# maybeLx/MVSFormerPlusPlus

Hardware: NVIDIA H100
Metric: depth-maps/sec (hot path: FMT + 4-stage cascade) (higher is better)
Workload: dtype f32

## Files before the change

mvsformerplusplus_b200/csrc/conv3d_tc.cu:

```cuda
#include "conv3d_tc.cuh"

#include <type_traits>

#include "linear_tc.cuh"
#include "wgmma.cuh"

namespace mvsf {

using namespace gmma;

namespace c3 {
constexpr int THREADS = 384, MAX_STAGES = 8;
template <int MODE, int NT>
struct Geo {
  static constexpr int TW = 8 * NT, TH = 16;
  static constexpr int PR = MODE == CONV_S1 ? TH + 2 : TH + 1;
  static constexpr int PC = MODE == CONV_S1 ? TW + 2 : TW + 1;
  static constexpr int NSUB = MODE == CONV_S2 ? 4 : 1;
  static constexpr uint32_t SUB_BYTES = PR * PC * 16;
  static constexpr uint32_t PAIR = (2 * SUB_BYTES + 127) / 128 * 128;
  static constexpr uint32_t OCT_BYTES = NSUB * PAIR;
  static constexpr uint32_t PITCH = PC * 16;
};
__host__ __device__ inline int npad(int cout) { return cout < 16 ? 16 : cout; }
__host__ __device__ inline uint32_t slab_bytes(int mode, int cout) { return (uint32_t)npad(cout) * (mode == DECONV_S2 ? 1024u : 576u); }

struct alignas(64) Maps { CUtensorMap m[4]; };
}

struct DepthTaps { int n, kd[3], id[3]; };
template <int MODE>
__device__ __forceinline__ DepthTaps depth_taps(int od, int SD, int ID) {
  DepthTaps t;
  t.n = 0;
#pragma unroll
  for (int kd = 0; kd < 3; ++kd) {
    int id;
    bool ok = true;
    if (MODE == CONV_S1) id = od + kd - 1;
    else if (MODE == CONV_S2) id = od * SD + kd - 1;
    else {
      const int num = od + 1 - kd;
      if (SD == 1) id = num;
      else { ok = (num & 1) == 0; id = num >> 1; }
    }
    if (ok && id >= 0 && id < ID) { t.kd[t.n] = kd; t.id[t.n] = id; ++t.n; }
  }
  return t;
}

template <int OUT, int NPAD>
__device__ __forceinline__ float conv_epilogue_frag(const ConvTcArgs& a, const float* acc, int h, int q, bool valid, size_t vox) {
  const int COUT = a.COUT;
  float prob = 0.f;
#pragma unroll
  for (int b = 0; b < NPAD / 8; ++b) {
    const int c = 8 * b + 2 * q;
    if (8 * b >= COUT) continue;
    const float2 b2 = *reinterpret_cast<const float2*>(a.bias + c);
    float x0 = fmaxf(acc[4 * b + 2 * h] + b2.x, 0.f), x1 = fmaxf(acc[4 * b + 2 * h + 1] + b2.y, 0.f);
    if (!valid) continue;
    if (OUT == OUT_SPLIT) {
      if (a.skip_hi) {
        const float2 fh = __half22float2(*reinterpret_cast<const __half2*>(a.skip_hi + vox * COUT + c));
        const float2 fl = __half22float2(*reinterpret_cast<const __half2*>(a.skip_lo + vox * COUT + c));
        x0 += fh.x + fl.x;
        x1 += fh.y + fl.y;
      }
      split_store2(a.out_hi + vox * COUT + c, a.out_lo + vox * COUT + c, x0, x1);
    } else {
      const float2 s2 = *reinterpret_cast<const float2*>(a.skip32 + vox * COUT + c);
      x0 += s2.x; x1 += s2.y;
      if (OUT == OUT_F32) *reinterpret_cast<float2*>(a.out32 + vox * COUT + c) = make_float2(x0, x1);
      else prob = fmaf(x1, __ldg(a.probw + c + 1), x0 * __ldg(a.probw + c));
    }
  }
  return prob;
}

template <int NREG>
__device__ __forceinline__ void fence_acc(float (&acc)[NREG]) { fence_regs<NREG>(acc); }

template <int MODE, int NT, int OUT, int NPAD>
__global__ void __launch_bounds__(c3::THREADS, 1)
conv3d_tc_kernel(const __grid_constant__ c3::Maps maps, ConvTcArgs a, int NS, int OD, int OH, int OW, int tiles_w,
                 int tiles_h, int ntiles) {
  using G = c3::Geo<MODE, NT>;
  constexpr int PC = G::PC, NSUB = G::NSUB;
  constexpr int NCLS = MODE == DECONV_S2 ? 4 : 1;
  constexpr int ACC = NCLS * NPAD / 2;
  extern __shared__ __align__(1024) unsigned char smem[];
  const int tid = threadIdx.x, warp = tid >> 5, lane = tid & 31;
  const int CIN = a.CIN, SD = a.SD, ID = a.ID, IH = a.IH, IW = a.IW;
  const int KG = a.KG;
  const uint32_t b_bytes = c3::slab_bytes(MODE, NPAD);
  const uint32_t a_bytes = (uint32_t)KG * G::OCT_BYTES;
  const uint32_t stage_bytes = (a_bytes + b_bytes + 127u) / 128u * 128u;
  const uint32_t sbase = smem_u32(smem);
  const uint32_t bars = sbase + NS * stage_bytes;
  const uint32_t bar_full = bars, bar_empty = bars + 64;
  const int ngroups = (CIN >> 3) / KG;

  if (tid == 0) {
    for (int i = 0; i < c3::MAX_STAGES; ++i) { mbar_init(bar_full + 8 * i, 1); mbar_init(bar_empty + 8 * i, 2); }
    fence_barrier_init();
  }
  __syncthreads();

  if (warp < 4) {
    asm volatile("setmaxnreg.dec.sync.aligned.u32 40;");
    if (tid == 0) {
      uint32_t g = 0;
      for (int tile = blockIdx.x; tile < ntiles; tile += gridDim.x) {
        const int tw = tile % tiles_w, th = (tile / tiles_w) % tiles_h, od = tile / (tiles_w * tiles_h);
        const int c0h = th * 16, c0w = tw * G::TW;
        const DepthTaps dt = depth_taps<MODE>(od, SD, ID);
        for (int ds = 0; ds < dt.n; ++ds) {
          for (int grp = 0; grp < ngroups; ++grp, ++g) {
            const int s = g % NS;
            mbar_wait(bar_empty + 8 * s, (uint32_t)(((g / NS) & 1) ^ 1));
            const uint32_t st = sbase + s * stage_bytes, full = bar_full + 8 * s;
            expect_tx(full, (uint32_t)(KG * NSUB) * 2u * G::SUB_BYTES + b_bytes);
            for (int og = 0; og < KG; ++og) {
              const int c = (grp * KG + og) * 8;
#pragma unroll
              for (int sub = 0; sub < NSUB; ++sub) {
// ... 50 lines not shown
        }
      };
      wg_fence();
      if constexpr (MODE == DECONV_S2) {
        issue(0u, 0, u == 0);
        issue(16u, 4, false);
        issue((uint32_t)PC * 16u, 8, false);
        issue((uint32_t)(PC + 1) * 16u, 12, false);
      } else {
#pragma unroll
        for (int kh = 0; kh < 3; ++kh) {
#pragma unroll
          for (int kw = 0; kw < 3; ++kw) {
            int sub = 0, rs = kh, cs = kw;
            if (MODE == CONV_S2) {
              sub = (kh == 1 ? 0 : 2) + (kw == 1 ? 0 : 1);
              rs = kh == 2 ? 1 : 0; cs = kw == 2 ? 1 : 0;
            }
            issue((uint32_t)sub * G::PAIR + (uint32_t)(rs * PC + cs) * 16u, kh * 3 + kw, u == 0 && kh == 0 && kw == 0);
          }
        }
      }
      wg_commit();
      if (pend >= 0) {
        wg_wait<1>();
        release((uint32_t)pend);
      }
      pend = (int)g;
    }
    wg_wait<0>();
#pragma unroll
    for (int t = 0; t < NT; ++t) fence_acc(acc[t]);
    release((uint32_t)pend);
#pragma unroll
    for (int t = 0; t < NT; ++t)
#pragma unroll
      for (int cls = 0; cls < NCLS; ++cls)
#pragma unroll
        for (int h = 0; h < 2; ++h) {
          const int ch = th * 16 + 8 * half + 2 * wq + h;
          const int cw = tw * G::TW + t * 8 + (lane >> 2);
          int oh, ow;
          bool valid;
          if (MODE == DECONV_S2) { oh = 2 * ch + (cls >> 1); ow = 2 * cw + (cls & 1); valid = ch < IH && cw < IW; }
          else { oh = ch; ow = cw; valid = ch < OH && cw < OW; }
          const size_t vox = valid ? ((size_t)od * OH + oh) * OW + ow : 0;
          float prob = conv_epilogue_frag<OUT, NPAD>(a, acc[t] + (cls ^ (cls >> 1)) * (NPAD / 2), h, q, valid, vox);
          if (OUT == OUT_PROB) {
            prob += __shfl_xor_sync(0xffffffffu, prob, 1);
            prob += __shfl_xor_sync(0xffffffffu, prob, 2);
            if (q == 0 && valid) a.out32[vox] = prob + __ldg(a.probw + a.COUT);
          }
        }
  }
}


template <int MODE, int NT, int NPAD>
__global__ void __launch_bounds__(c3::THREADS, 1)
conv3d_col_kernel(const __grid_constant__ c3::Maps maps, ConvTcArgs a, int NS, int wres, int OH, int OW, int tiles_w,
                  int tiles_h, int DC, int nitems) {
  using G = c3::Geo<MODE, NT>;
  constexpr int PC = G::PC, NSUB = G::NSUB;
  extern __shared__ __align__(1024) unsigned char smem[];
  const int tid = threadIdx.x, warp = tid >> 5, lane = tid & 31;
  const int CIN = a.CIN, D = a.ID;
  const int KG = a.KG;
  const int ngroups = (CIN >> 3) / KG;
  const uint32_t slab = (uint32_t)NPAD * 1728u;
  const uint32_t a_bytes = (uint32_t)KG * G::OCT_BYTES;
  const uint32_t stage_bytes = (a_bytes + (wres ? 0u : slab) + 127u) / 128u * 128u;
  const uint32_t sbase = smem_u32(smem);
  const uint32_t wbase = sbase;
  const uint32_t ring = sbase + (wres ? ((uint32_t)ngroups * slab + 127u) / 128u * 128u : 0u);
  const uint32_t bars = ring + NS * stage_bytes;
  const uint32_t bar_full = bars, bar_empty = bars + 64, bar_w = bars + 128;

  if (tid == 0) {
    for (int i = 0; i < c3::MAX_STAGES; ++i) { mbar_init(bar_full + 8 * i, 1); mbar_init(bar_empty + 8 * i, 2); }
    mbar_init(bar_w, 1);
    fence_barrier_init();
  }
  __syncthreads();
  const int tiles_hw = tiles_w * tiles_h;

  if (warp < 4) {
    asm volatile("setmaxnreg.dec.sync.aligned.u32 40;");
    if (tid == 0) {
      if (wres) {
        expect_tx(bar_w, (uint32_t)ngroups * slab);
        for (int grp = 0; grp < ngroups; ++grp) bulk_load(wbase + grp * slab, a.wtc + (size_t)grp * (slab / 2), slab, bar_w);
      }
      uint32_t g = 0;
      for (int item = blockIdx.x; item < nitems; item += gridDim.x) {
        const int tw = item % tiles_w, th = (item / tiles_w) % tiles_h, ck = item / tiles_hw;
        const int c0h = th * 16, c0w = tw * G::TW;
        const int d0 = ck * DC, d1 = min(D, d0 + DC);
        const int first_id = max(d0 - 1, 0), last_id = min(d1, D - 1);
        for (int id = first_id; id <= last_id; ++id) {
          for (int grp = 0; grp < ngroups; ++grp, ++g) {
            const int s = g % NS;
            mbar_wait(bar_empty + 8 * s, (uint32_t)(((g / NS) & 1) ^ 1));
            const uint32_t st = ring + s * stage_bytes, full = bar_full + 8 * s;
            expect_tx(full, (uint32_t)(KG * NSUB) * 2u * G::SUB_BYTES + (wres ? 0u : slab));
            for (int og = 0; og < KG; ++og) {
              const int c = (grp * KG + og) * 8;
#pragma unroll
              for (int sub = 0; sub < NSUB; ++sub) {
                int w0, h0;
                if (MODE == CONV_S1) { w0 = c0w - 1; h0 = c0h - 1; }
                else { w0 = c0w - (sub & 1); h0 = c0h - (sub >> 1); }
                tma_load_5d(st + (uint32_t)(og * NSUB + sub) * G::PAIR, &maps.m[sub], c, w0, h0, id, 0, full);
              }
            }
            if (!wres) bulk_load(st + a_bytes, a.wtc + (size_t)grp * (slab / 2), slab, full);
          }
        }
      }
    }
    return;
  }
  asm volatile("setmaxnreg.inc.sync.aligned.u32 232;");
  const int half = (warp >> 2) - 1, wq = warp & 3, q = lane & 3, t128 = tid & 127;
  if (wres) mbar_wait(bar_w, 0u);
  constexpr uint32_t btile = (uint32_t)NPAD * 96u;
  constexpr uint32_t blbo = (uint32_t)NPAD * 48u;
  constexpr int SL = NPAD / 2;
  float acc[NT][3 * SL];
  auto release = [&](uint32_t gb) { if (t128 == 0) mbar_arrive(bar_empty + 8 * (gb % NS)); };
  auto epilogue = [&](int od, int th, int tw, auto third_c) {
#pragma unroll
    for (int t = 0; t < NT; ++t)
#pragma unroll
      for (int h = 0; h < 2; ++h) {
        const int ch = th * 16 + 8 * half + 2 * wq + h;
        const int cw = tw * G::TW + t * 8 + (lane >> 2);
        const bool valid = ch < OH && cw < OW;
        const size_t vox = valid ? ((size_t)od * OH + ch) * OW + cw : 0;
        conv_epilogue_frag<OUT_SPLIT, NPAD>(a, acc[t] + decltype(third_c)::value * SL, h, q, valid, vox);
      }
  };
  uint32_t g = 0;
  for (int item = blockIdx.x; item < nitems; item += gridDim.x) {
    const int tw = item % tiles_w, th = (item / tiles_w) % tiles_h, ck = item / tiles_hw;
    const int d0 = ck * DC, d1 = min(D, d0 + DC);
    const int first_id = max(d0 - 1, 0), last_id = min(d1, D - 1);
#pragma unroll
    for (int t = 0; t < NT; ++t)
#pragma unroll
      for (int i = 0; i < 3 * SL; ++i) acc[t][i] = 0.f;
    for (int id = first_id; id <= last_id; ++id) {
      int pend = -1;
      for (int grp = 0; grp < ngroups; ++grp, ++g) {
        const int s = g % NS;
        mbar_wait(bar_full + 8 * s, (uint32_t)((g / NS) & 1));
        const uint32_t sA = ring + s * stage_bytes + (uint32_t)half * 8u * G::PITCH;
        const uint32_t sB = wres ? wbase + grp * slab : ring + s * stage_bytes + a_bytes;
        wg_fence();
#pragma unroll
        for (int kh = 0; kh < 3; ++kh) {
#pragma unroll
          for (int kw = 0; kw < 3; ++kw) {
            int sub = 0, rs = kh, cs = kw;
            if (MODE == CONV_S2) {
              sub = (kh == 1 ? 0 : 2) + (kw == 1 ? 0 : 1);
              rs = kh == 2 ? 1 : 0; cs = kw == 2 ? 1 : 0;
            }
            const uint32_t aoff = sA + (uint32_t)sub * G::PAIR + (uint32_t)(rs * PC + cs) * 16u;
            const uint32_t t0 = sB + (uint32_t)(kh * 3 + kw) * 2u * btile, t1 = t0 + btile;
            const uint32_t va[3] = {KG == 1 ? aoff : aoff + G::SUB_BYTES, KG == 1 ? aoff : aoff, aoff};
            const uint32_t vl = KG == 1 ? G::SUB_BYTES : G::OCT_BYTES;
            const uint32_t vt[3] = {t0, t1, t0};
            const int nv = KG == 1 ? 2 : 3;
#pragma unroll
            for (int v = 0; v < 3; ++v) {
              if (v >= nv) break;
              const uint64_t bd = make_desc(vt[v], blbo, 128);
#pragma unroll
              for (int t = 0; t < NT; ++t) mma_ss<3 * NPAD>(acc[t], make_desc(va[v] + t * 128, vl, G::PITCH), bd, 1u);
            }
          }
        }
        wg_commit();
        if (pend >= 0) {
          wg_wait<1>();
          release((uint32_t)pend);
        }
        pend = (int)g;
      }
      wg_wait<0>();
#pragma unroll
      for (int t = 0; t < NT; ++t) fence_acc(acc[t]);
      release((uint32_t)pend);
      if (id - 1 >= d0) epilogue(id - 1, th, tw, std::integral_constant<int, 0>{});
      if (id == last_id && id <= d1 - 1) epilogue(id, th, tw, std::integral_constant<int, 1>{});
#pragma unroll
      for (int t = 0; t < NT; ++t)
#pragma unroll
        for (int i = 0; i < SL; ++i) {
          acc[t][i] = acc[t][SL + i];
          acc[t][SL + i] = acc[t][2 * SL + i];
          acc[t][2 * SL + i] = 0.f;
        }
    }
  }
}

int conv3d_tc_kg(int mode, int cin) { return (mode != CONV_S2 && cin >= 16) ? 2 : 1; }
int conv3d_tc_col(int mode, int sd, int cout) { return (mode == CONV_S1 || (mode == CONV_S2 && sd == 1)) && c3::npad(cout) <= 32; }

size_t conv3d_tc_packed_halves(int mode, int cin, int cout) {
  return (size_t)3 * (cin / 8 / conv3d_tc_kg(mode, cin)) * (c3::slab_bytes(mode, cout) / 2);
}

__global__ void conv3d_tc_pack_kernel(const float* __restrict__ w32, __half* __restrict__ out, int cin, int cout, int NPAD,
                                      int KG, int deconv, int col, size_t total) {
  size_t i = (size_t)blockIdx.x * blockDim.x + threadIdx.x;
  if (i >= total) return;
  const int e = (int)(i & 7);
  const size_t q = i >> 3;
  const int per_slab = col ? NPAD * 108 : (deconv ? NPAD * 64 : NPAD * 36);
  const int slab = (int)(q / per_slab), c = (int)(q % per_slab);
  const int ngroups = cin / 8 / KG;
  int kd = slab / ngroups, g = slab % ngroups;
  int mm, kc, n, kh = 0, kw = 0;
  bool tap = true;
  if (col) {
    g = slab;
    n = c % NPAD;
    int r = c / NPAD;
    kd = 2 - r % 3; r /= 3;
    kc = r & 1; r >>= 1;
    mm = r & 1; r >>= 1;
    kh = r / 3; kw = r % 3;
  } else if (!deconv) {
    n = c % NPAD;
    int r = c / NPAD;
    kc = r & 1; r >>= 1;
    mm = r & 1; r >>= 1;
    kh = r / 3; kw = r % 3;
  } else {
    const int tkh[4][4] = {{1, 1, 2, 2}, {-1, 1, 2, -1}, {-1, -1, 0, 0}, {-1, -1, 0, -1}};
    const int tkw[4][4] = {{1, 2, 2, 1}, {-1, 0, 0, -1}, {-1, -1, 2, 1}, {-1, -1, 0, -1}};
    const int t = c / (16 * NPAD), cc = c % (16 * NPAD);
    mm = cc / (8 * NPAD);
    kc = (cc / (4 * NPAD)) & 1;
    const int nn = cc % (4 * NPAD);
    const int b = nn / NPAD;
    n = nn % NPAD;
    kh = tkh[t][b]; kw = tkw[t][b];
    tap = kh >= 0;
  }
  const int ci = (KG == 1 ? g : g * 2 + kc) * 8 + e;
  float w = 0.f;
  if (tap && n < cout) w = w32[((size_t)((kd * 3 + kh) * 3 + kw) * cin + ci) * cout + n];
  __half hi, lo;
  split_f16(w, hi, lo);
  __half v;
  if (KG == 1) v = mm == 0 ? hi : (kc == 0 ? lo : __float2half_rn(0.f));
  else v = mm == 0 ? hi : lo;
  out[i] = v;
}

int conv3d_tc_pack(const float* w32, __half* out, int mode, int sd, int cin, int cout, cudaStream_t s) {
  MVSF_REQUIRE(w32 && out && cin % 8 == 0 && cout % 8 == 0, "conv3d_tc_pack: bad arguments");
  const size_t total = conv3d_tc_packed_halves(mode, cin, cout);
  conv3d_tc_pack_kernel<<<cdiv((long long)total, 256), 256, 0, s>>>(w32, out, cin, cout, c3::npad(cout),
                                                                     conv3d_tc_kg(mode, cin), mode == DECONV_S2 ? 1 : 0,
                                                                     conv3d_tc_col(mode, sd, cout), total);
  MVSF_LAUNCH_CHECK("conv3d_tc_pack");
  return MVSF_OK;
}

__global__ void merge_vec8_kernel(const __half* __restrict__ hi, const __half* __restrict__ lo, float* __restrict__ x, size_t n8) {
  size_t i = (size_t)blockIdx.x * blockDim.x + threadIdx.x;
  if (i >= n8) return;
// ... 82 lines not shown
  else { OD = a.ID * a.SD; OH = a.IH * 2; OW = a.IW * 2; cells_h = a.IH; cells_w = a.IW; }
  const int num_sms = device_sm_count(current_device());
  const int NPAD = c3::npad(a.COUT);
  const uint32_t b_bytes = c3::slab_bytes(MODE, a.COUT);
  const int ncls = MODE == DECONV_S2 ? 4 : 1;
  int best_nt = 0;
  double best_eff = -1.0;
  const int nts[3] = {4, 2, 1};
  size_t stage_of[5] = {0, 0, 0, 0, 0};
  for (int k = 0; k < 3; ++k) {
    const int nt = nts[k];
    const uint32_t oct = nt == 4 ? c3::Geo<MODE, 4>::OCT_BYTES : (nt == 2 ? c3::Geo<MODE, 2>::OCT_BYTES : c3::Geo<MODE, 1>::OCT_BYTES);
    const size_t stage = align_up((size_t)a.KG * oct + b_bytes, 128);
    stage_of[nt] = stage;
    if (nt * ncls * NPAD > 256 || 2 * stage + 256 > 227 * 1024) continue;
    const long long ntiles = (long long)cdiv(cells_w, 8 * nt) * cdiv(cells_h, 16) * OD;
    const double eff = (double)ntiles / (double)(cdiv(ntiles, num_sms) * (long long)num_sms);
    if (eff >= 0.85) { best_nt = nt; break; }
    if (eff > best_eff) { best_eff = eff; best_nt = nt; }
  }
  MVSF_REQUIRE(best_nt > 0, "conv3d_tc: no tile shape fits (COUT %d)", a.COUT);
  const size_t stage = stage_of[best_nt];
  int NS = (int)((227 * 1024 - 256) / stage);
  if (NS > c3::MAX_STAGES) NS = c3::MAX_STAGES;
  const size_t smem = NS * stage + 256;
  if constexpr (OUT == OUT_SPLIT) {
    if (NPAD == 32) return launch_nt<MODE, OUT, 32>(a, best_nt, NS, smem, OD, OH, OW, cells_h, cells_w, num_sms, s);
    if (NPAD == 64) return launch_nt<MODE, OUT, 64>(a, best_nt, NS, smem, OD, OH, OW, cells_h, cells_w, num_sms, s);
  }
  return launch_nt<MODE, OUT, 16>(a, best_nt, NS, smem, OD, OH, OW, cells_h, cells_w, num_sms, s);
}


template <int MODE, int NT, int NPAD>
static int launch_col_one(const ConvTcArgs& a, int NS, int wres, size_t smem, int OH, int OW, int DC, int num_sms, cudaStream_t s) {
  using G = c3::Geo<MODE, NT>;
  auto kern = conv3d_col_kernel<MODE, NT, NPAD>;
  static DeviceOnce once;
  const int dev = current_device();
  if (once.need(dev)) {
    MVSF_CUDA_OK(cudaFuncSetAttribute(kern, cudaFuncAttributeMaxDynamicSharedMemorySize, 227 * 1024));
    once.done(dev);
  }
  c3::Maps maps;
  int rc;
  if (MODE == CONV_S2) {
    for (int sub = 0; sub < 4; ++sub)
      if ((rc = make_map(&maps.m[sub], a.in_hi, a.in_lo, a.CIN, a.ID, a.IH, a.IW, 2, 2, sub >> 1, sub & 1, G::PC, G::PR))) return rc;
  } else {
    if ((rc = make_map(&maps.m[0], a.in_hi, a.in_lo, a.CIN, a.ID, a.IH, a.IW, 1, 1, 0, 0, G::PC, G::PR))) return rc;
    maps.m[1] = maps.m[2] = maps.m[3] = maps.m[0];
  }
  const int tiles_w = cdiv(OW, 8 * NT), tiles_h = cdiv(OH, 16);
  const long long nitems = (long long)tiles_w * tiles_h * cdiv(a.ID, DC);
  MVSF_REQUIRE(nitems < (1ll << 30), "conv3d_tc: volume too large");
  const int grid = (int)(nitems < num_sms ? nitems : num_sms);
  kern<<<grid, c3::THREADS, smem, s>>>(maps, a, NS, wres, OH, OW, tiles_w, tiles_h, DC, (int)nitems);
  MVSF_LAUNCH_CHECK("conv3d_col");
  return MVSF_OK;
}

template <int MODE>
static int launch_col(const ConvTcArgs& a, cudaStream_t s) {
  const int D = a.ID;
  const int OH = MODE == CONV_S1 ? a.IH : (a.IH - 1) / 2 + 1, OW = MODE == CONV_S1 ? a.IW : (a.IW - 1) / 2 + 1;
  const int num_sms = device_sm_count(current_device());
  const int NPAD = c3::npad(a.COUT);
  const int ngroups = a.CIN / 8 / a.KG;
  const size_t slab = (size_t)NPAD * 1728;
  const size_t wres_bytes = align_up(ngroups * slab, 128);
  const int wres = wres_bytes <= 112 * 1024 ? 1 : 0;
  int best_nt = 0, best_dc = 0, best_ns = 0;
  size_t best_smem = 0;
  double best_cost = 1e30;
  const int nts[3] = {4, 2, 1};
  for (int k = 0; k < 3; ++k) {
    const int nt = nts[k];
    if (3 * nt * NPAD > 128) continue;
    const uint32_t oct = nt == 4 ? c3::Geo<MODE, 4>::OCT_BYTES : (nt == 2 ? c3::Geo<MODE, 2>::OCT_BYTES : c3::Geo<MODE, 1>::OCT_BYTES);
    const size_t stage = align_up((size_t)a.KG * oct + (wres ? 0 : slab), 128);
    const size_t fixed = (wres ? wres_bytes : 0) + 256;
    int ns = (int)((227 * 1024 - fixed) / stage);
    if (ns > c3::MAX_STAGES) ns = c3::MAX_STAGES;
    if (ns < 2) continue;
    for (int div = 1; div <= 8; div *= 2) {
      const int dc = cdiv(D, div);
      if (div > 1 && dc == cdiv(D, div / 2)) continue;
      const long long items = (long long)cdiv(OW, 8 * nt) * cdiv(OH, 16) * cdiv(D, dc);
      const double eff = (double)items / (double)(cdiv(items, num_sms) * (long long)num_sms);
      const double halo_w = MODE == CONV_S1 ? (8.0 * nt + 2) / (8.0 * nt) : (16.0 * nt + 1) / (16.0 * nt);
      const double halo_d = dc >= D ? 1.0 : (dc + 2.0) / dc;
      const double cost = halo_w * halo_d / eff;
      if (cost < best_cost) { best_cost = cost; best_nt = nt; best_dc = dc; best_ns = ns; best_smem = fixed + ns * stage; }
    }
  }
  MVSF_REQUIRE(best_nt > 0, "conv3d_col: no tile shape fits (CIN %d COUT %d)", a.CIN, a.COUT);
  if (NPAD == 16) {
    if (best_nt == 2) return launch_col_one<MODE, 2, 16>(a, best_ns, wres, best_smem, OH, OW, best_dc, num_sms, s);
    return launch_col_one<MODE, 1, 16>(a, best_ns, wres, best_smem, OH, OW, best_dc, num_sms, s);
  }
  return launch_col_one<MODE, 1, 32>(a, best_ns, wres, best_smem, OH, OW, best_dc, num_sms, s);
}

int launch_conv3d_tc(const ConvTcArgs& a, int mode, int out_mode, cudaStream_t s) {
  MVSF_REQUIRE(a.in_hi && a.in_lo && a.wtc && a.bias, "conv3d_tc: null pointer");
  MVSF_REQUIRE(a.CIN % 8 == 0 && a.CIN >= 8 && a.CIN <= 64 && (a.COUT == 8 || a.COUT == 16 || a.COUT == 32 || a.COUT == 64),
               "conv3d_tc: input channels must be a multiple of 8 up to 64, output channels 8, 16, 32 or 64");
  MVSF_REQUIRE(a.SD == 1 || a.SD == 2, "conv3d_tc: depth stride must be 1 or 2");
  MVSF_REQUIRE(a.KG == conv3d_tc_kg(mode, a.CIN), "conv3d_tc: KG must be conv3d_tc_kg(mode, CIN) (it fixes the weight slab layout)");
  MVSF_REQUIRE(((uintptr_t)a.in_hi & 15) == 0 && ((uintptr_t)a.in_lo & 15) == 0 && ((uintptr_t)a.wtc & 15) == 0,
               "conv3d_tc: operands must be 16-byte aligned");
  MVSF_REQUIRE(a.col == conv3d_tc_col(mode, a.SD, a.COUT), "conv3d_tc: col must be conv3d_tc_col(mode, SD, COUT) (weight slab layout)");
  if (out_mode == OUT_SPLIT) {
    MVSF_REQUIRE(a.out_hi && a.out_lo, "conv3d_tc: split output missing");
    if (a.col) return mode == CONV_S1 ? launch_col<CONV_S1>(a, s) : launch_col<CONV_S2>(a, s);
    if (mode == CONV_S1) return launch_mode<CONV_S1, OUT_SPLIT>(a, s);
    if (mode == CONV_S2) return launch_mode<CONV_S2, OUT_SPLIT>(a, s);
    if (mode == DECONV_S2) return launch_mode<DECONV_S2, OUT_SPLIT>(a, s);
  } else if (mode == DECONV_S2 && (out_mode == OUT_F32 || out_mode == OUT_PROB)) {
    MVSF_REQUIRE(a.out32 && a.skip32 && a.COUT == 8 && (out_mode == OUT_F32 || a.probw), "conv3d_tc: fp32 output needs out32, skip32, COUT == 8");
    if (out_mode == OUT_F32) return launch_mode<DECONV_S2, OUT_F32>(a, s);
    return launch_mode<DECONV_S2, OUT_PROB>(a, s);
  }
  return fail(MVSF_ERR_INVALID, "conv3d_tc: unsupported mode %d / output %d", mode, out_mode);
}

}

using namespace mvsf;

extern "C" int mvsf_conv3d_tc_layer(int mode, int sd, const float* in, const float* w32, const float* skip, float* out,
                                    void* workspace, size_t workspace_bytes, int cin, int cout, int ID, int IH, int IW,
                                    mvsf_stream_t stream) {
  MVSF_REQUIRE(in && w32 && out && workspace && (mode >= 0 && mode <= 2) && (sd == 1 || sd == 2), "conv3d_tc_layer: bad arguments");
  MVSF_REQUIRE(cin % 8 == 0 && cout % 8 == 0, "conv3d_tc_layer: channels must be multiples of 8");
  int OD, OH, OW;
  if (mode == CONV_S1) { OD = ID; OH = IH; OW = IW; }
  else if (mode == CONV_S2) { OD = (ID - 1) / sd + 1; OH = (IH - 1) / 2 + 1; OW = (IW - 1) / 2 + 1; }
  else { OD = ID * sd; OH = IH * 2; OW = IW * 2; }
  const size_t nin = (size_t)ID * IH * IW * cin, nout = (size_t)OD * OH * OW * cout;
  const size_t nw = align_up(conv3d_tc_packed_halves(mode, cin, cout), 64);
  const size_t need = (2 * nin + 4 * nout + nw) * sizeof(__half) + 256;
  if (workspace_bytes < need) return fail(MVSF_ERR_WORKSPACE, "conv3d_tc_layer: workspace %zu < %zu bytes", workspace_bytes, need);
  cudaStream_t s = (cudaStream_t)stream;
  __half* xin = reinterpret_cast<__half*>(workspace);
  __half* xout = xin + 2 * nin;
  __half* xskip = xout + 2 * nout;
  __half* wtc = xskip + 2 * nout;
  int rc;
  if ((rc = launch_split_f16(in, nin, xin, 2 * nin, 1, nin, s))) return rc;
  if (skip && (rc = launch_split_f16(skip, nout, xskip, 2 * nout, 1, nout, s))) return rc;
  if ((rc = conv3d_tc_pack(w32, wtc, mode, sd, cin, cout, s))) return rc;
  ConvTcArgs a{};
  a.in_hi = xin; a.in_lo = xin + nin; a.wtc = wtc; a.bias = w32 + (size_t)27 * cin * cout;
  if (skip) { a.skip_hi = xskip; a.skip_lo = xskip + nout; }
// ... 7 lines not shown
```

mvsformerplusplus_b200/csrc/costreg_unet.cu:

```cuda
#include "common.cuh"
#include "conv3d_tc.cuh"

namespace mvsf {

__global__ void prob3_kernel(const float* __restrict__ in, const float* __restrict__ w, float* __restrict__ out, int D,
                             int H, int W) {
  __shared__ float ws[27 * 8];
  for (int i = threadIdx.x; i < 27 * 8; i += blockDim.x) ws[i] = __ldg(w + i);
  __syncthreads();
  int x = blockIdx.x * blockDim.x + threadIdx.x, y = blockIdx.y, d = blockIdx.z;
  if (x >= W) return;
  float acc = 0.f;
  for (int kd = 0; kd < 3; ++kd) {
    int zd = d + kd - 1;
    if (zd < 0 || zd >= D) continue;
    for (int kh = 0; kh < 3; ++kh) {
      int yh = y + kh - 1;
      if (yh < 0 || yh >= H) continue;
#pragma unroll
      for (int kw = 0; kw < 3; ++kw) {
        int xw = x + kw - 1;
        if (xw < 0 || xw >= W) continue;
        const float* p = in + (((size_t)zd * H + yh) * W + xw) * 8;
        float4 a = ldg4(p), b = ldg4(p + 4);
// ... 47 lines not shown
      p += kLayerCh[l][1];
      q += conv3d_tc_packed_halves(kLayerMode[l], kLayerCh[l][0], kLayerCh[l][1]);
    }
  }
  const float* wp = bias[8] + 8;
  int rc;
  if ((rc = launch_split_f16(vol, n0, v0, 2 * n0, 1, n0, s))) return rc;
  auto conv = [&](int l, const __half* in, size_t nin, __half* out, size_t nout, const __half* skip, size_t nskip,
                  int ID, int IH, int IW) {
    ConvTcArgs a{};
    a.in_hi = in; a.in_lo = in + nin;
    a.wtc = w16[l]; a.bias = bias[l];
    a.skip_hi = skip; a.skip_lo = skip ? skip + nskip : nullptr;
    a.out_hi = out; a.out_lo = out + nout;
    a.CIN = kLayerCh[l][0]; a.COUT = kLayerCh[l][1]; a.SD = SD; a.ID = ID; a.IH = IH; a.IW = IW;
    a.KG = conv3d_tc_kg(kLayerMode[l], a.CIN);
    a.col = conv3d_tc_col(kLayerMode[l], SD, a.COUT);
    return launch_conv3d_tc(a, kLayerMode[l], OUT_SPLIT, s);
  };
  if ((rc = conv(0, v0, n0, t1, n1, nullptr, 0, D, H, W))) return rc;
  if ((rc = conv(1, t1, n1, c2, n1, nullptr, 0, D1, H1, W1))) return rc;
  if ((rc = conv(2, c2, n1, t3, n2, nullptr, 0, D1, H1, W1))) return rc;
  if ((rc = conv(3, t3, n2, c4, n2, nullptr, 0, D2, H2, W2))) return rc;
  if ((rc = conv(4, c4, n2, t5, n3, nullptr, 0, D2, H2, W2))) return rc;
  if ((rc = conv(5, t5, n3, c6, n3, nullptr, 0, D3, H3, W3))) return rc;
  if ((rc = conv(6, c6, n3, t3, n2, c4, n2, D3, H3, W3))) return rc;
  if ((rc = conv(7, t3, n2, t1, n1, c2, n1, D2, H2, W2))) return rc;
  {
    ConvTcArgs a{};
    a.in_hi = t1; a.in_lo = t1 + n1;
    a.wtc = w16[8]; a.bias = bias[8];
    a.skip32 = vol;
    a.CIN = 16; a.COUT = 8; a.SD = SD; a.ID = D1; a.IH = H1; a.IW = W1; a.KG = conv3d_tc_kg(DECONV_S2, 16);
    if (kind == 1) {
      a.out32 = logits; a.probw = wp;
      if ((rc = launch_conv3d_tc(a, DECONV_S2, OUT_PROB, s))) return rc;
    } else {
      a.out32 = x11;
      if ((rc = launch_conv3d_tc(a, DECONV_S2, OUT_F32, s))) return rc;
      dim3 grid(cdiv(W, 128), H, D);
      prob3_kernel<<<grid, 128, 0, s>>>(x11, wp, logits, D, H, W);
      MVSF_LAUNCH_CHECK("prob3");
    }
  }
  return MVSF_OK;
}

}

using namespace mvsf;

extern "C" {

int mvsf_costreg_unet_workspace_bytes(int kind, int C, int D, int H, int W, size_t* bytes) {
  MVSF_REQUIRE(bytes && (kind == 0 || kind == 1) && C == 8, "costreg_unet: kind in {0,1}, C == 8");
  MVSF_REQUIRE(H % 8 == 0 && W % 8 == 0 && D >= 1 && (kind == 1 || D % 8 == 0),
               "costreg_unet: H, W (and D for CostRegNet) must be multiples of 8");
  const int SD = kind == 0 ? 2 : 1;
  size_t D1 = (D - 1) / SD + 1, D2 = (D1 - 1) / SD + 1, D3 = (D2 - 1) / SD + 1;
  size_t n1 = D1 * (H / 2) * (W / 2) * 16, n2 = D2 * (H / 4) * (W / 4) * 32, n3 = D3 * (H / 8) * (W / 8) * 64;
  size_t n = (size_t)D * H * W * 8 + 2 * (n1 + n2 + n3) + (kind == 0 ? (size_t)D * H * W * 8 : 0);
  *bytes = n * sizeof(float);
  return MVSF_OK;
}

int mvsf_costreg_unet_tc_bytes(size_t* bytes) {
// ... 35 lines not shown
```

Before: 51.03.

## Run depth-stride-1 deconv with fused prob epilogue on column kernel

Extends the depth-column conv kernel to the transposed stride-2 conv (DECONV_S2) with depth stride 1, packing all three depth taps for the four output phases into one weight slab so each input depth slice is loaded once and reused across output depths. Depth iteration runs in reverse for deconv. The epilogue of one finished output plane is deferred into registers and overlapped with the next slice's async MMAs, with skip loads preloaded. It costs extra registers and a new weight-packing layout.

```diff
diff --git a/mvsformerplusplus_b200/csrc/conv3d_tc.cu b/mvsformerplusplus_b200/csrc/conv3d_tc.cu
--- a/mvsformerplusplus_b200/csrc/conv3d_tc.cu
+++ b/mvsformerplusplus_b200/csrc/conv3d_tc.cu
@@ -24,6 +24,7 @@
 };
 __host__ __device__ inline int npad(int cout) { return cout < 16 ? 16 : cout; }
 __host__ __device__ inline uint32_t slab_bytes(int mode, int cout) { return (uint32_t)npad(cout) * (mode == DECONV_S2 ? 1024u : 576u); }
+__host__ __device__ constexpr uint32_t col_slab_bytes(int mode, int npad) { return (uint32_t)npad * (mode == DECONV_S2 ? 3072u : 1728u); }
 
 struct alignas(64) Maps { CUtensorMap m[4]; };
 }
@@ -50,7 +51,28 @@
 }
 
 template <int OUT, int NPAD>
-__device__ __forceinline__ float conv_epilogue_frag(const ConvTcArgs& a, const float* acc, int h, int q, bool valid, size_t vox) {
+__device__ __forceinline__ void conv_epilogue_skip(const ConvTcArgs& a, int q, bool valid, size_t vox, float2 (&sk)[NPAD / 8]) {
+  const int COUT = a.COUT;
+#pragma unroll
+  for (int b = 0; b < NPAD / 8; ++b) {
+    const int c = 8 * b + 2 * q;
+    sk[b] = make_float2(0.f, 0.f);
+    if (8 * b >= COUT || !valid) continue;
+    if (OUT == OUT_SPLIT) {
+      if (a.skip_hi) {
+        const float2 fh = __half22float2(*reinterpret_cast<const __half2*>(a.skip_hi + vox * COUT + c));
+        const float2 fl = __half22float2(*reinterpret_cast<const __half2*>(a.skip_lo + vox * COUT + c));
+        sk[b] = make_float2(fh.x + fl.x, fh.y + fl.y);
+      }
+    } else {
+      sk[b] = *reinterpret_cast<const float2*>(a.skip32 + vox * COUT + c);
+    }
+  }
+}
+
+template <int OUT, int NPAD, bool PRE>
+__device__ __forceinline__ float conv_epilogue_frag(const ConvTcArgs& a, const float* acc, int h, int q, bool valid, size_t vox,
+                                                    const float2* sk) {
   const int COUT = a.COUT;
   float prob = 0.f;
 #pragma unroll
@@ -62,20 +84,74 @@
     if (!valid) continue;
     if (OUT == OUT_SPLIT) {
       if (a.skip_hi) {
-        const float2 fh = __half22float2(*reinterpret_cast<const __half2*>(a.skip_hi + vox * COUT + c));
-        const float2 fl = __half22float2(*reinterpret_cast<const __half2*>(a.skip_lo + vox * COUT + c));
-        x0 += fh.x + fl.x;
-        x1 += fh.y + fl.y;
+        if (PRE) {
+          x0 += sk[b].x;
+          x1 += sk[b].y;
+        } else {
+          const float2 fh = __half22float2(*reinterpret_cast<const __half2*>(a.skip_hi + vox * COUT + c));
+          const float2 fl = __half22float2(*reinterpret_cast<const __half2*>(a.skip_lo + vox * COUT + c));
+          x0 += fh.x + fl.x;
+          x1 += fh.y + fl.y;
+        }
       }
       split_store2(a.out_hi + vox * COUT + c, a.out_lo + vox * COUT + c, x0, x1);
     } else {
-      const float2 s2 = *reinterpret_cast<const float2*>(a.skip32 + vox * COUT + c);
+      const float2 s2 = PRE ? sk[b] : *reinterpret_cast<const float2*>(a.skip32 + vox * COUT + c);
       x0 += s2.x; x1 += s2.y;
       if (OUT == OUT_F32) *reinterpret_cast<float2*>(a.out32 + vox * COUT + c) = make_float2(x0, x1);
       else prob = fmaf(x1, __ldg(a.probw + c + 1), x0 * __ldg(a.probw + c));
     }
   }
   return prob;
+}
+
+template <int MODE>
+__device__ __forceinline__ bool conv_epilogue_cell(const ConvTcArgs& a, int cls, int h, int od, int ch0, int cw, int OH, int OW,
+                                                   size_t& vox) {
+  const int ch = ch0 + h;
+  int oh, ow;
+  bool valid;
+  if (MODE == DECONV_S2) { oh = 2 * ch + (cls >> 1); ow = 2 * cw + (cls & 1); valid = ch < a.IH && cw < a.IW; }
+  else { oh = ch; ow = cw; valid = ch < OH && cw < OW; }
+  vox = valid ? ((size_t)od * OH + oh) * OW + ow : 0;
+  return valid;
+}
+
+template <int MODE, int NPAD>
+struct EpiSkip { float2 v[MODE == DECONV_S2 ? 4 : 1][2][NPAD / 8]; };
+
+template <int MODE, int OUT, int NPAD>
+__device__ __forceinline__ void conv_epilogue_preload(const ConvTcArgs& a, int od, int ch0, int cw, int OH, int OW, int q,
+                                                      EpiSkip<MODE, NPAD>& sk) {
+  constexpr int NCLS = MODE == DECONV_S2 ? 4 : 1;
+#pragma unroll
+  for (int cls = 0; cls < NCLS; ++cls)
+#pragma unroll
+    for (int h = 0; h < 2; ++h) {
+      size_t vox;
+      const bool valid = conv_epilogue_cell<MODE>(a, cls, h, od, ch0, cw, OH, OW, vox);
+      conv_epilogue_skip<OUT, NPAD>(a, q, valid, vox, sk.v[cls][h]);
+    }
+}
+
+template <int MODE, int OUT, int NPAD, bool PRE>
+__device__ __forceinline__ void conv_epilogue_tile(const ConvTcArgs& a, const float* acc, int od, int ch0, int cw, int OH,
+                                                   int OW, int q, const EpiSkip<MODE, NPAD>* sk) {
+  constexpr int NCLS = MODE == DECONV_S2 ? 4 : 1;
+#pragma unroll
+  for (int cls = 0; cls < NCLS; ++cls)
+#pragma unroll
+    for (int h = 0; h < 2; ++h) {
+      size_t vox;
+      const bool valid = conv_epilogue_cell<MODE>(a, cls, h, od, ch0, cw, OH, OW, vox);
+      float prob = conv_epilogue_frag<OUT, NPAD, PRE>(a, acc + (cls ^ (cls >> 1)) * (NPAD / 2), h, q, valid, vox,
+                                                      PRE ? sk->v[cls][h] : nullptr);
+      if (OUT == OUT_PROB) {
+        prob += __shfl_xor_sync(0xffffffffu, prob, 1);
+        prob += __shfl_xor_sync(0xffffffffu, prob, 2);
+        if (q == 0 && valid) a.out32[vox] = prob + __ldg(a.probw + a.COUT);
+      }
+    }
 }
 
 template <int NREG>
@@ -85,13 +161,14 @@
 __global__ void __launch_bounds__(c3::THREADS, 1)
 conv3d_tc_kernel(const __grid_constant__ c3::Maps maps, ConvTcArgs a, int NS, int OD, int OH, int OW, int tiles_w,
                  int tiles_h, int ntiles) {
+  static_assert(OUT != OUT_PROB, "the fused prob epilogue runs on conv3d_col_kernel");
   using G = c3::Geo<MODE, NT>;
   constexpr int PC = G::PC, NSUB = G::NSUB;
   constexpr int NCLS = MODE == DECONV_S2 ? 4 : 1;
   constexpr int ACC = NCLS * NPAD / 2;
   extern __shared__ __align__(1024) unsigned char smem[];
   const int tid = threadIdx.x, warp = tid >> 5, lane = tid & 31;
-  const int CIN = a.CIN, SD = a.SD, ID = a.ID, IH = a.IH, IW = a.IW;
+  const int CIN = a.CIN, SD = a.SD, ID = a.ID;
   const int KG = a.KG;
   const uint32_t b_bytes = c3::slab_bytes(MODE, NPAD);
   const uint32_t a_bytes = (uint32_t)KG * G::OCT_BYTES;
@@ -208,42 +285,32 @@
 #pragma unroll
     for (int t = 0; t < NT; ++t) fence_acc(acc[t]);
     release((uint32_t)pend);
-#pragma unroll
-    for (int t = 0; t < NT; ++t)
-#pragma unroll
-      for (int cls = 0; cls < NCLS; ++cls)
-#pragma unroll
-        for (int h = 0; h < 2; ++h) {
-          const int ch = th * 16 + 8 * half + 2 * wq + h;
-          const int cw = tw * G::TW + t * 8 + (lane >> 2);
-          int oh, ow;
-          bool valid;
-          if (MODE == DECONV_S2) { oh = 2 * ch + (cls >> 1); ow = 2 * cw + (cls & 1); valid = ch < IH && cw < IW; }
-          else { oh = ch; ow = cw; valid = ch < OH && cw < OW; }
-          const size_t vox = valid ? ((size_t)od * OH + oh) * OW + ow : 0;
-          float prob = conv_epilogue_frag<OUT, NPAD>(a, acc[t] + (cls ^ (cls >> 1)) * (NPAD / 2), h, q, valid, vox);
-          if (OUT == OUT_PROB) {
-            prob += __shfl_xor_sync(0xffffffffu, prob, 1);
-            prob += __shfl_xor_sync(0xffffffffu, prob, 2);
-            if (q == 0 && valid) a.out32[vox] = prob + __ldg(a.probw + a.COUT);
-          }
-        }
-  }
-}
-
-
-template <int MODE, int NT, int NPAD>
+    constexpr bool PRE = MODE == DECONV_S2 && NPAD == 16;
+#pragma unroll
+    for (int t = 0; t < NT; ++t) {
+      const int ch0 = th * 16 + 8 * half + 2 * wq, cw = tw * G::TW + t * 8 + (lane >> 2);
+      EpiSkip<MODE, NPAD> sk;
+      if (PRE) conv_epilogue_preload<MODE, OUT, NPAD>(a, od, ch0, cw, OH, OW, q, sk);
+      conv_epilogue_tile<MODE, OUT, NPAD, PRE>(a, acc[t], od, ch0, cw, OH, OW, q, &sk);
+    }
+  }
+}
+
+
+template <int MODE, int NT, int OUT, int NPAD>
 __global__ void __launch_bounds__(c3::THREADS, 1)
 conv3d_col_kernel(const __grid_constant__ c3::Maps maps, ConvTcArgs a, int NS, int wres, int OH, int OW, int tiles_w,
                   int tiles_h, int DC, int nitems) {
   using G = c3::Geo<MODE, NT>;
   constexpr int PC = G::PC, NSUB = G::NSUB;
+  constexpr int NCLS = MODE == DECONV_S2 ? 4 : 1;
+  constexpr int STEP = MODE == DECONV_S2 ? -1 : 1;
   extern __shared__ __align__(1024) unsigned char smem[];
   const int tid = threadIdx.x, warp = tid >> 5, lane = tid & 31;
   const int CIN = a.CIN, D = a.ID;
   const int KG = a.KG;
   const int ngroups = (CIN >> 3) / KG;
-  const uint32_t slab = (uint32_t)NPAD * 1728u;
+  constexpr uint32_t slab = c3::col_slab_bytes(MODE, NPAD);
   const uint32_t a_bytes = (uint32_t)KG * G::OCT_BYTES;
   const uint32_t stage_bytes = (a_bytes + (wres ? 0u : slab) + 127u) / 128u * 128u;
   const uint32_t sbase = smem_u32(smem);
@@ -272,8 +339,9 @@
         const int tw = item % tiles_w, th = (item / tiles_w) % tiles_h, ck = item / tiles_hw;
         const int c0h = th * 16, c0w = tw * G::TW;
         const int d0 = ck * DC, d1 = min(D, d0 + DC);
-        const int first_id = max(d0 - 1, 0), last_id = min(d1, D - 1);
-        for (int id = first_id; id <= last_id; ++id) {
+        const int lo_id = max(d0 - 1, 0), hi_id = min(d1, D - 1);
+        for (int k = 0; k <= hi_id - lo_id; ++k) {
+          const int id = STEP > 0 ? lo_id + k : hi_id - k;
           for (int grp = 0; grp < ngroups; ++grp, ++g) {
             const int s = g % NS;
             mbar_wait(bar_empty + 8 * s, (uint32_t)(((g / NS) & 1) ^ 1));
@@ -285,7 +353,8 @@
               for (int sub = 0; sub < NSUB; ++sub) {
                 int w0, h0;
                 if (MODE == CONV_S1) { w0 = c0w - 1; h0 = c0h - 1; }
-                else { w0 = c0w - (sub & 1); h0 = c0h - (sub >> 1); }
+                else if (MODE == CONV_S2) { w0 = c0w - (sub & 1); h0 = c0h - (sub >> 1); }
+                else { w0 = c0w; h0 = c0h; }
                 tma_load_5d(st + (uint32_t)(og * NSUB + sub) * G::PAIR, &maps.m[sub], c, w0, h0, id, 0, full);
               }
             }
@@ -299,65 +368,85 @@
   asm volatile("setmaxnreg.inc.sync.aligned.u32 232;");
   const int half = (warp >> 2) - 1, wq = warp & 3, q = lane & 3, t128 = tid & 127;
   if (wres) mbar_wait(bar_w, 0u);
-  constexpr uint32_t btile = (uint32_t)NPAD * 96u;
-  constexpr uint32_t blbo = (uint32_t)NPAD * 48u;
-  constexpr int SL = NPAD / 2;
+  constexpr uint32_t btile = (uint32_t)(NCLS * NPAD) * 96u;
+  constexpr uint32_t blbo = (uint32_t)(NCLS * NPAD) * 48u;
+  constexpr int SL = NCLS * NPAD / 2;
   float acc[NT][3 * SL];
+  constexpr bool OVERLAP = MODE == DECONV_S2;
+  float ep[OVERLAP ? NT : 1][SL];
+  int ep_od = -1, ep_th = 0, ep_tw = 0;
   auto release = [&](uint32_t gb) { if (t128 == 0) mbar_arrive(bar_empty + 8 * (gb % NS)); };
-  auto epilogue = [&](int od, int th, int tw, auto third_c) {
-#pragma unroll
-    for (int t = 0; t < NT; ++t)
-#pragma unroll
-      for (int h = 0; h < 2; ++h) {
-        const int ch = th * 16 + 8 * half + 2 * wq + h;
-        const int cw = tw * G::TW + t * 8 + (lane >> 2);
-        const bool valid = ch < OH && cw < OW;
-        const size_t vox = valid ? ((size_t)od * OH + ch) * OW + cw : 0;
-        conv_epilogue_frag<OUT_SPLIT, NPAD>(a, acc[t] + decltype(third_c)::value * SL, h, q, valid, vox);
-      }
+  const int ch_w = 8 * half + 2 * wq, cw_l = lane >> 2;
+  auto epilogue = [&](const float* src, int tstride, int od, int th, int tw) {
+#pragma unroll
+    for (int t = 0; t < NT; ++t) {
+      const int ch0 = th * 16 + ch_w, cw = tw * G::TW + t * 8 + cw_l;
+      EpiSkip<MODE, NPAD> sk;
+      if (OVERLAP) conv_epilogue_preload<MODE, OUT, NPAD>(a, od, ch0, cw, OH, OW, q, sk);
+      conv_epilogue_tile<MODE, OUT, NPAD, OVERLAP>(a, src + t * tstride, od, ch0, cw, OH, OW, q, &sk);
+    }
   };
+  auto epilogue_ep = [&]() { epilogue(&ep[0][0], SL, ep_od, ep_th, ep_tw); };
   uint32_t g = 0;
   for (int item = blockIdx.x; item < nitems; item += gridDim.x) {
     const int tw = item % tiles_w, th = (item / tiles_w) % tiles_h, ck = item / tiles_hw;
     const int d0 = ck * DC, d1 = min(D, d0 + DC);
-    const int first_id = max(d0 - 1, 0), last_id = min(d1, D - 1);
+    const int lo_id = max(d0 - 1, 0), hi_id = min(d1, D - 1);
 #pragma unroll
     for (int t = 0; t < NT; ++t)
 #pragma unroll
       for (int i = 0; i < 3 * SL; ++i) acc[t][i] = 0.f;
-    for (int id = first_id; id <= last_id; ++id) {
+    for (int k = 0; k <= hi_id - lo_id; ++k) {
+      const int id = STEP > 0 ? lo_id + k : hi_id - k;
       int pend = -1;
       for (int grp = 0; grp < ngroups; ++grp, ++g) {
         const int s = g % NS;
         mbar_wait(bar_full + 8 * s, (uint32_t)((g / NS) & 1));
         const uint32_t sA = ring + s * stage_bytes + (uint32_t)half * 8u * G::PITCH;
         const uint32_t sB = wres ? wbase + grp * slab : ring + s * stage_bytes + a_bytes;
+        auto tap = [&](uint32_t aoff, int j) {
+          const uint32_t t0 = sB + (uint32_t)j * 2u * btile, t1 = t0 + btile;
+          const uint32_t va[3] = {KG == 1 ? aoff : aoff + G::SUB_BYTES, KG == 1 ? aoff : aoff, aoff};
+          const uint32_t vl = KG == 1 ? G::SUB_BYTES : G::OCT_BYTES;
+          const uint32_t vt[3] = {t0, t1, t0};
+          const int nv = KG == 1 ? 2 : 3;
+#pragma unroll
+          for (int v = 0; v < 3; ++v) {
+            if (v >= nv) break;
+            const uint64_t bd = make_desc(vt[v], blbo, 128);
+#pragma unroll
+            for (int t = 0; t < NT; ++t) mma_ss<3 * NCLS * NPAD>(acc[t], make_desc(va[v] + t * 128, vl, G::PITCH), bd, 1u);
+          }
+        };
         wg_fence();
-#pragma unroll
-        for (int kh = 0; kh < 3; ++kh) {
-#pragma unroll
-          for (int kw = 0; kw < 3; ++kw) {
-            int sub = 0, rs = kh, cs = kw;
-            if (MODE == CONV_S2) {
-              sub = (kh == 1 ? 0 : 2) + (kw == 1 ? 0 : 1);
-              rs = kh == 2 ? 1 : 0; cs = kw == 2 ? 1 : 0;
-            }
-            const uint32_t aoff = sA + (uint32_t)sub * G::PAIR + (uint32_t)(rs * PC + cs) * 16u;
-            const uint32_t t0 = sB + (uint32_t)(kh * 3 + kw) * 2u * btile, t1 = t0 + btile;
-            const uint32_t va[3] = {KG == 1 ? aoff : aoff + G::SUB_BYTES, KG == 1 ? aoff : aoff, aoff};
-            const uint32_t vl = KG == 1 ? G::SUB_BYTES : G::OCT_BYTES;
-            const uint32_t vt[3] = {t0, t1, t0};
-            const int nv = KG == 1 ? 2 : 3;
-#pragma unroll
-            for (int v = 0; v < 3; ++v) {
-              if (v >= nv) break;
-              const uint64_t bd = make_desc(vt[v], blbo, 128);
-#pragma unroll
-              for (int t = 0; t < NT; ++t) mma_ss<3 * NPAD>(acc[t], make_desc(va[v] + t * 128, vl, G::PITCH), bd, 1u);
+        if constexpr (MODE == DECONV_S2) {
+          tap(sA, 0);
+          tap(sA + 16u, 1);
+          tap(sA + (uint32_t)PC * 16u, 2);
+          tap(sA + (uint32_t)(PC + 1) * 16u, 3);
+        } else {
+#pragma unroll
+          for (int kh = 0; kh < 3; ++kh) {
+#pragma unroll
+            for (int kw = 0; kw < 3; ++kw) {
+              int sub = 0, rs = kh, cs = kw;
+              if (MODE == CONV_S2) {
+                sub = (kh == 1 ? 0 : 2) + (kw == 1 ? 0 : 1);
+                rs = kh == 2 ? 1 : 0; cs = kw == 2 ? 1 : 0;
+              }
+              tap(sA + (uint32_t)sub * G::PAIR + (uint32_t)(rs * PC + cs) * 16u, kh * 3 + kw);
             }
           }
         }
         wg_commit();
+        if constexpr (OVERLAP) {
+          if (grp == 0) {
+            if (ep_od >= 0) {
+              epilogue_ep();
+              ep_od = -1;
+            }
+          }
+        }
         if (pend >= 0) {
           wg_wait<1>();
           release((uint32_t)pend);
@@ -368,8 +457,20 @@
 #pragma unroll
       for (int t = 0; t < NT; ++t) fence_acc(acc[t]);
       release((uint32_t)pend);
-      if (id - 1 >= d0) epilogue(id - 1, th, tw, std::integral_constant<int, 0>{});
-      if (id == last_id && id <= d1 - 1) epilogue(id, th, tw, std::integral_constant<int, 1>{});
+      const bool done0 = id - STEP >= d0 && id - STEP < d1, done1 = k == hi_id - lo_id && id >= d0 && id < d1;
+      if constexpr (OVERLAP) {
+        if (done1) epilogue(&acc[0][SL], 3 * SL, id, th, tw);
+        if (done0) {
+#pragma unroll
+          for (int t = 0; t < NT; ++t)
+#pragma unroll
+            for (int i = 0; i < SL; ++i) ep[t][i] = acc[t][i];
+          ep_od = id - STEP; ep_th = th; ep_tw = tw;
+        }
+      } else {
+        if (done0) epilogue(&acc[0][0], 3 * SL, id - STEP, th, tw);
+        if (done1) epilogue(&acc[0][SL], 3 * SL, id, th, tw);
+      }
 #pragma unroll
       for (int t = 0; t < NT; ++t)
 #pragma unroll
@@ -380,10 +481,14 @@
         }
     }
   }
+  if (OVERLAP && ep_od >= 0) epilogue_ep();
 }
 
 int conv3d_tc_kg(int mode, int cin) { return (mode != CONV_S2 && cin >= 16) ? 2 : 1; }
-int conv3d_tc_col(int mode, int sd, int cout) { return (mode == CONV_S1 || (mode == CONV_S2 && sd == 1)) && c3::npad(cout) <= 32; }
+int conv3d_tc_col(int mode, int sd, int cout) {
+  if (mode == DECONV_S2) return sd == 1 && c3::npad(cout) == 16;
+  return (mode == CONV_S1 || sd == 1) && c3::npad(cout) <= 32;
+}
 
 size_t conv3d_tc_packed_halves(int mode, int cin, int cout) {
   return (size_t)3 * (cin / 8 / conv3d_tc_kg(mode, cin)) * (c3::slab_bytes(mode, cout) / 2);
@@ -395,13 +500,25 @@
   if (i >= total) return;
   const int e = (int)(i & 7);
   const size_t q = i >> 3;
-  const int per_slab = col ? NPAD * 108 : (deconv ? NPAD * 64 : NPAD * 36);
+  const int per_slab = col ? (deconv ? NPAD * 192 : NPAD * 108) : (deconv ? NPAD * 64 : NPAD * 36);
   const int slab = (int)(q / per_slab), c = (int)(q % per_slab);
   const int ngroups = cin / 8 / KG;
   int kd = slab / ngroups, g = slab % ngroups;
   int mm, kc, n, kh = 0, kw = 0;
   bool tap = true;
-  if (col) {
+  const int tkh[4][4] = {{1, 1, 2, 2}, {-1, 1, 2, -1}, {-1, -1, 0, 0}, {-1, -1, 0, -1}};
+  const int tkw[4][4] = {{1, 2, 2, 1}, {-1, 0, 0, -1}, {-1, -1, 2, 1}, {-1, -1, 0, -1}};
+  if (col && deconv) {
+    g = slab;
+    n = c % NPAD;
+    int r = c / NPAD;
+    const int b = r % 4; r /= 4;
+    kd = 2 - r % 3; r /= 3;
+    kc = r & 1; r >>= 1;
+    mm = r & 1; r >>= 1;
+    kh = tkh[r][b]; kw = tkw[r][b];
+    tap = kh >= 0;
+  } else if (col) {
     g = slab;
     n = c % NPAD;
     int r = c / NPAD;
@@ -416,8 +533,6 @@
     mm = r & 1; r >>= 1;
     kh = r / 3; kw = r % 3;
   } else {
-    const int tkh[4][4] = {{1, 1, 2, 2}, {-1, 1, 2, -1}, {-1, -1, 0, 0}, {-1, -1, 0, -1}};
-    const int tkw[4][4] = {{1, 2, 2, 1}, {-1, 0, 0, -1}, {-1, -1, 2, 1}, {-1, -1, 0, -1}};
     const int t = c / (16 * NPAD), cc = c % (16 * NPAD);
     mm = cc / (8 * NPAD);
     kc = (cc / (4 * NPAD)) & 1;
@@ -566,10 +681,11 @@
 }
 
 
-template <int MODE, int NT, int NPAD>
-static int launch_col_one(const ConvTcArgs& a, int NS, int wres, size_t smem, int OH, int OW, int DC, int num_sms, cudaStream_t s) {
+template <int MODE, int NT, int OUT, int NPAD>
+static int launch_col_one(const ConvTcArgs& a, int NS, int wres, size_t smem, int OH, int OW, int cells_h, int cells_w,
+                          int DC, int num_sms, cudaStream_t s) {
   using G = c3::Geo<MODE, NT>;
-  auto kern = conv3d_col_kernel<MODE, NT, NPAD>;
+  auto kern = conv3d_col_kernel<MODE, NT, OUT, NPAD>;
   static DeviceOnce once;
   const int dev = current_device();
   if (once.need(dev)) {
@@ -585,7 +701,7 @@
     if ((rc = make_map(&maps.m[0], a.in_hi, a.in_lo, a.CIN, a.ID, a.IH, a.IW, 1, 1, 0, 0, G::PC, G::PR))) return rc;
     maps.m[1] = maps.m[2] = maps.m[3] = maps.m[0];
   }
-  const int tiles_w = cdiv(OW, 8 * NT), tiles_h = cdiv(OH, 16);
+  const int tiles_w = cdiv(cells_w, 8 * NT), tiles_h = cdiv(cells_h, 16);
   const long long nitems = (long long)tiles_w * tiles_h * cdiv(a.ID, DC);
   MVSF_REQUIRE(nitems < (1ll << 30), "conv3d_tc: volume too large");
   const int grid = (int)(nitems < num_sms ? nitems : num_sms);
@@ -594,14 +710,17 @@
   return MVSF_OK;
 }
 
-template <int MODE>
+template <int MODE, int OUT>
 static int launch_col(const ConvTcArgs& a, cudaStream_t s) {
   const int D = a.ID;
-  const int OH = MODE == CONV_S1 ? a.IH : (a.IH - 1) / 2 + 1, OW = MODE == CONV_S1 ? a.IW : (a.IW - 1) / 2 + 1;
+  int OH, OW, cells_h, cells_w;
+  if (MODE == CONV_S1) { OH = a.IH; OW = a.IW; cells_h = OH; cells_w = OW; }
+  else if (MODE == CONV_S2) { OH = (a.IH - 1) / 2 + 1; OW = (a.IW - 1) / 2 + 1; cells_h = OH; cells_w = OW; }
+  else { OH = 2 * a.IH; OW = 2 * a.IW; cells_h = a.IH; cells_w = a.IW; }
   const int num_sms = device_sm_count(current_device());
   const int NPAD = c3::npad(a.COUT);
   const int ngroups = a.CIN / 8 / a.KG;
-  const size_t slab = (size_t)NPAD * 1728;
+  const size_t slab = c3::col_slab_bytes(MODE, NPAD);
   const size_t wres_bytes = align_up(ngroups * slab, 128);
   const int wres = wres_bytes <= 112 * 1024 ? 1 : 0;
   int best_nt = 0, best_dc = 0, best_ns = 0;
@@ -610,7 +729,7 @@
   const int nts[3] = {4, 2, 1};
   for (int k = 0; k < 3; ++k) {
     const int nt = nts[k];
-    if (3 * nt * NPAD > 128) continue;
+    if (MODE == DECONV_S2 ? nt != 1 : 3 * nt * NPAD > 128) continue;
     const uint32_t oct = nt == 4 ? c3::Geo<MODE, 4>::OCT_BYTES : (nt == 2 ? c3::Geo<MODE, 2>::OCT_BYTES : c3::Geo<MODE, 1>::OCT_BYTES);
     const size_t stage = align_up((size_t)a.KG * oct + (wres ? 0 : slab), 128);
     const size_t fixed = (wres ? wres_bytes : 0) + 256;
@@ -620,20 +739,26 @@
     for (int div = 1; div <= 8; div *= 2) {
       const int dc = cdiv(D, div);
       if (div > 1 && dc == cdiv(D, div / 2)) continue;
-      const long long items = (long long)cdiv(OW, 8 * nt) * cdiv(OH, 16) * cdiv(D, dc);
+      const long long items = (long long)cdiv(cells_w, 8 * nt) * cdiv(cells_h, 16) * cdiv(D, dc);
       const double eff = (double)items / (double)(cdiv(items, num_sms) * (long long)num_sms);
-      const double halo_w = MODE == CONV_S1 ? (8.0 * nt + 2) / (8.0 * nt) : (16.0 * nt + 1) / (16.0 * nt);
+      const double halo_w = MODE == CONV_S1 ? (8.0 * nt + 2) / (8.0 * nt) : MODE == CONV_S2 ? (16.0 * nt + 1) / (16.0 * nt)
+                                                                                             : (8.0 * nt + 1) / (8.0 * nt);
       const double halo_d = dc >= D ? 1.0 : (dc + 2.0) / dc;
       const double cost = halo_w * halo_d / eff;
       if (cost < best_cost) { best_cost = cost; best_nt = nt; best_dc = dc; best_ns = ns; best_smem = fixed + ns * stage; }
     }
   }
   MVSF_REQUIRE(best_nt > 0, "conv3d_col: no tile shape fits (CIN %d COUT %d)", a.CIN, a.COUT);
-  if (NPAD == 16) {
-    if (best_nt == 2) return launch_col_one<MODE, 2, 16>(a, best_ns, wres, best_smem, OH, OW, best_dc, num_sms, s);
-    return launch_col_one<MODE, 1, 16>(a, best_ns, wres, best_smem, OH, OW, best_dc, num_sms, s);
-  }
-  return launch_col_one<MODE, 1, 32>(a, best_ns, wres, best_smem, OH, OW, best_dc, num_sms, s);
+  if constexpr (MODE == DECONV_S2) {
+    return launch_col_one<MODE, 1, OUT, 16>(a, best_ns, wres, best_smem, OH, OW, cells_h, cells_w, best_dc, num_sms, s);
+  } else {
+    static_assert(OUT == OUT_SPLIT, "convolutions write fp16 hi|lo activations");
+    if (NPAD == 16) {
+      if (best_nt == 2) return launch_col_one<MODE, 2, OUT, 16>(a, best_ns, wres, best_smem, OH, OW, cells_h, cells_w, best_dc, num_sms, s);
+      return launch_col_one<MODE, 1, OUT, 16>(a, best_ns, wres, best_smem, OH, OW, cells_h, cells_w, best_dc, num_sms, s);
+    }
+    return launch_col_one<MODE, 1, OUT, 32>(a, best_ns, wres, best_smem, OH, OW, cells_h, cells_w, best_dc, num_sms, s);
+  }
 }
 
 int launch_conv3d_tc(const ConvTcArgs& a, int mode, int out_mode, cudaStream_t s) {
@@ -647,14 +772,19 @@
   MVSF_REQUIRE(a.col == conv3d_tc_col(mode, a.SD, a.COUT), "conv3d_tc: col must be conv3d_tc_col(mode, SD, COUT) (weight slab layout)");
   if (out_mode == OUT_SPLIT) {
     MVSF_REQUIRE(a.out_hi && a.out_lo, "conv3d_tc: split output missing");
-    if (a.col) return mode == CONV_S1 ? launch_col<CONV_S1>(a, s) : launch_col<CONV_S2>(a, s);
+    if (a.col) {
+      if (mode == CONV_S1) return launch_col<CONV_S1, OUT_SPLIT>(a, s);
+      if (mode == CONV_S2) return launch_col<CONV_S2, OUT_SPLIT>(a, s);
+      return launch_col<DECONV_S2, OUT_SPLIT>(a, s);
+    }
     if (mode == CONV_S1) return launch_mode<CONV_S1, OUT_SPLIT>(a, s);
     if (mode == CONV_S2) return launch_mode<CONV_S2, OUT_SPLIT>(a, s);
     if (mode == DECONV_S2) return launch_mode<DECONV_S2, OUT_SPLIT>(a, s);
   } else if (mode == DECONV_S2 && (out_mode == OUT_F32 || out_mode == OUT_PROB)) {
     MVSF_REQUIRE(a.out32 && a.skip32 && a.COUT == 8 && (out_mode == OUT_F32 || a.probw), "conv3d_tc: fp32 output needs out32, skip32, COUT == 8");
+    MVSF_REQUIRE(a.col == (out_mode == OUT_PROB), "conv3d_tc: the fp32 output needs depth stride 2, the fused prob output depth stride 1");
     if (out_mode == OUT_F32) return launch_mode<DECONV_S2, OUT_F32>(a, s);
-    return launch_mode<DECONV_S2, OUT_PROB>(a, s);
+    return launch_col<DECONV_S2, OUT_PROB>(a, s);
   }
   return fail(MVSF_ERR_INVALID, "conv3d_tc: unsupported mode %d / output %d", mode, out_mode);
 }
diff --git a/mvsformerplusplus_b200/csrc/costreg_unet.cu b/mvsformerplusplus_b200/csrc/costreg_unet.cu
--- a/mvsformerplusplus_b200/csrc/costreg_unet.cu
+++ b/mvsformerplusplus_b200/csrc/costreg_unet.cu
@@ -103,6 +103,7 @@
     a.wtc = w16[8]; a.bias = bias[8];
     a.skip32 = vol;
     a.CIN = 16; a.COUT = 8; a.SD = SD; a.ID = D1; a.IH = H1; a.IW = W1; a.KG = conv3d_tc_kg(DECONV_S2, 16);
+    a.col = conv3d_tc_col(DECONV_S2, SD, a.COUT);
     if (kind == 1) {
       a.out32 = logits; a.probw = wp;
       if ((rc = launch_conv3d_tc(a, DECONV_S2, OUT_PROB, s))) return rc;
```

After: 52.36, median of 6. 1.03x the previous value.
